# orybkin/video-gcp

Hardware: AMD Instinct MI355X
Metric: predicted frames/sec, 64x64x3 seq_len=80 gcp_tree (posterior forward + all loss terms, model(inputs) and model.loss() of train.py:157-159, batch-stat BatchNorm) (higher is better)
Workload: dtype f32 (encoder / decoder convs and the tree GEMMs from 512 rows: split-f16 MFMA with f32 accumulate, f32-equivalent; everything else exact f32 MFMA)

## Files before the change

include/gcpx.h:

```cpp
#ifndef GCPX_H
#define GCPX_H

#include <stdint.h>

#ifdef __cplusplus
extern "C" {
#endif

#define GCPX_VERSION 1

typedef enum gcpx_status {
    GCPX_OK = 0,
    GCPX_ERR_INVALID_ARG = -1,
    GCPX_ERR_UNSUPPORTED = -2,
    GCPX_ERR_HIP = -3,
    GCPX_ERR_COMM = -4
} gcpx_status;

typedef enum gcpx_act { GCPX_ACT_NONE = 0, GCPX_ACT_LRELU = 1, GCPX_ACT_TANH = 2 } gcpx_act;

int gcpx_version(void);
const char* gcpx_last_error(void);
int gcpx_conv_grid(void);

typedef struct gcpx_conv_src {
    const float* ptr;
    const float* scale;
    const float* shift;
    int32_t C;
    int32_t frame_div;
    int32_t act;
    int32_t _pad;
} gcpx_conv_src;

typedef enum gcpx_head_mode {
    GCPX_HEAD_RAW = 0,
    GCPX_HEAD_DLM_MEAN = 1,
    GCPX_HEAD_DLM_BOTH = 2,
    GCPX_HEAD_TANH_NCHW = 3,
    GCPX_HEAD_DLM_NLL = 4,
    GCPX_HEAD_DLM_NLL_GRAD = 5
} gcpx_head_mode;

typedef struct gcpx_conv_args {
    gcpx_conv_src src[2];
    int32_t nsrc;
    int32_t F;
    int32_t Hin, Win;
    int32_t Hout, Wout;
    int32_t Cin;
    int32_t Cout;
    int32_t out_pitch;
    int32_t upsample;
    int32_t out_act;
    int32_t head_mode;
    const float* wpk;
    const float* bias;
    float* out;
    float* images;
    float* stats_partial;
    const int32_t* raw_row_map;
    const int32_t* src_row_map;
    const int32_t* src_row_frames;
    int32_t n_src_rows;
    int32_t w_split_log2;
    const void* wpk_split;
    const int32_t* w_split_log2_dev;
    int32_t split_layout;
    int32_t nll_rows;
    const float* nll_target;
    float* nll_partial;
    const float* nll_row_weight;
    float nll_scale;
    int32_t _pad3;
    float* images_rows;
    int64_t images_rows_dup;
    const float* bwd_r;
    const float *bwd_scale, *bwd_shift, *bwd_mean, *bwd_rstd;
    const float* addend;
    int32_t addend_frame_div;
    int32_t _pad4;
} gcpx_conv_args;

typedef enum gcpx_split_layout { GCPX_SPLIT_PLAIN = 0, GCPX_SPLIT_ROWFOLD = 1, GCPX_SPLIT_HEAD32 = 2 } gcpx_split_layout;

int gcpx_conv3x3(const gcpx_conv_args* a, void* stream);
int gcpx_conv3x3_grid(const gcpx_conv_args* a);
int gcpx_conv4x4s2(const gcpx_conv_args* a, void* stream);
int gcpx_conv4x4s2_grid(void);
int gcpx_conv4x4s2_image(const float* x, const float* wpk, const float* bias, float* out,
                         int32_t F, int32_t Hin, int32_t Win, int32_t Cout, int32_t out_act, void* stream);

int gcpx_bn_finalize(const float* partial, int32_t n_partial, int32_t pitch, int32_t C, double count,
                     const float* gamma, const float* beta, float eps, float* scale, float* shift,
                     float* running_mean, float* running_var, float momentum, float* mean_out, float* rstd_out,
                     void* stream);
int gcpx_randn(float* out, int64_t n, uint64_t* state, void* stream);
int gcpx_bn_fold(const float* running_mean, const float* running_var, const float* gamma, const float* beta,
                 float eps, int32_t C, float* scale, float* shift, void* stream);

typedef struct gcpx_row_src {
    const float* ptr;
    const int32_t* rowidx;
    const float* scale;
    const float* shiftv;
    int64_t sb, sr;
    int32_t width;
    int32_t shift;
    int32_t act;
    int32_t cmod;
} gcpx_row_src;

typedef enum gcpx_gemm_epi {
    GCPX_EPI_NONE = 0,
    GCPX_EPI_LRELU = 1,
    GCPX_EPI_LSTM = 2,
    GCPX_EPI_GAUSS_SAMPLE = 3
} gcpx_gemm_epi;

struct gcpx_lstm_bwd_args;
typedef struct gcpx_gemm_args {
    gcpx_row_src src[6];
    int32_t nsrc;
    int32_t M, N, K, rpb;
    const float* wpk;
    const float* bias;
    float* out;
    int64_t ob, orow;
    int32_t epi;
    int32_t nbatch;
    float* stats_partial;
    const float* c_prev;
    int64_t c_prev_stride;
    float* h_out;
    float* c_out;
    int64_t hb, hrow;
    float* h_copy;
    int64_t z_src_off, z_w_off, z_bias_off, z_out_off;
    float* gates_out;
    const void* wpk_split;
    const int32_t* w_split_log2_dev;
    int32_t w_split_log2;
    int32_t _pad_split;
    void* x_planes;
    int32_t* x_exp;
    int64_t x_planes_bytes;
    const struct gcpx_lstm_bwd_args* lstm_bwd;
} gcpx_gemm_args;

int gcpx_gemm(const gcpx_gemm_args* a, void* stream);
int gcpx_gemm_planes_workspace(int32_t M, int32_t K, int32_t nbatch, int64_t* planes_bytes, int64_t* n_exp);
int gcpx_gemm_group_dims(const gcpx_gemm_args* host_table, int32_t n, int32_t* dims, int32_t* total_blocks);
int gcpx_gemm_group(const gcpx_gemm_args* dev_table, const int32_t* dev_dims, int32_t n, int32_t total_blocks, void* stream);
int gcpx_gemm_row_blocks(int32_t M, int32_t N);

typedef enum gcpx_mlp_epi { GCPX_MLP_PLAIN = 0, GCPX_MLP_GAUSS = 1,
                             GCPX_MLP_TANH = 2  } gcpx_mlp_epi;

typedef struct gcpx_mlp_args {
    gcpx_row_src src[6];
    int32_t nsrc;
    int32_t M, rpb;
    int32_t in_dim, mid, n_mid, out_dim;
    const float* w_in;
    const float* b_in;
    const float* w_mid;
    const float* b_mid;
    const float* gn_gamma;
    const float* gn_beta;
    const float* w_out;
    const float* b_out;
    float gn_eps;
    float lrelu_slope;
    int32_t epi;
// ... 420 lines not shown
```

video-gcp_amd/forward_plan.py:

```python
import ctypes as C
import os
from contextlib import contextmanager

import torch

from . import packing as pk
from . import runtime as rt
from .hparams import GCPHParams
from .params import init_params, encoder_layers, encoder_skip_layers, decoder_layers
from .plan_ops import _Plan, _addr, N_LANES


class ForwardPlanMixin:

    def _plan_encoder(self, plan, tag, x_ptr, F, out_ptr, out_ob, out_orow, out_rpb):
        hp, P, lib = self._hp, self.pk, self.lib
        G = lib.gcpx_conv4x4s2_grid()
        S = hp.img_sz
        skip_idx = encoder_skip_layers(hp)
        skips = {}
        a0 = self._buf(f"{tag}.a0", (F, S // 2, S // 2, hp.ngf))
        enc_rec = dict(F=F, x_ptr=x_ptr, a0=a0, r={}, out=(out_ptr, out_ob, out_orow, out_rpb))
        plan.rec[f"enc:{tag}"] = enc_rec
        plan.add(f"enc.input:{tag}", lib.gcpx_conv4x4s2_image, x_ptr, P["enc.input.w"].data_ptr(),
                 P["enc.input.b"].data_ptr(), a0.data_ptr(), F, S, S, hp.ngf, rt.ACT_LRELU)
        prev = (a0.data_ptr(), hp.ngf, 1, None, None, rt.ACT_NONE)
        if 0 in skip_idx:
            skips[0] = (a0, hp.ngf, None, None, rt.ACT_NONE)
        res = S // 2
        for li, (name, cin, cout, norm) in enumerate(self._enc_layers[1:], start=1):
            r = self._buf(f"{tag}.r{li}", (F, res // 2, res // 2, cout))
            enc_rec["r"][li] = r
            stats = self._buf(f"{tag}.st{li}", (G, 2, cout)) if self.training else None
            a = self._conv_args([prev], F, res, res, res // 2, res // 2, cout, cout, P[f"enc.{name}.w"],
                                P[f"enc.{name}.b"], r, stats=stats)
            self._set_split(a, f"enc.{name}")
            plan.keep.append(a)
            plan.add(f"enc.{name}:{tag}", lib.gcpx_conv4x4s2, C.byref(a))
            res //= 2
            scale, shift = self._bn(plan, f"{tag}.bn{li}", f"encoder.net.{name}.norm", cout, stats, G, cout,
                                    F * res * res)
            prev = (r.data_ptr(), cout, 1, scale, shift, rt.ACT_LRELU)
            if li in skip_idx:
                skips[li] = (r, cout, scale, shift, rt.ACT_LRELU)
        assert res == 4
        ctop = self._c_top
        src = self._rowsrc(prev[0], 16 * ctop, 16 * ctop, 16 * ctop, scale=prev[3], shiftv=prev[4], act=prev[5], cmod=ctop)
        src.sb, src.sr = out_rpb * 16 * ctop, 16 * ctop
        self._gemm(plan, f"enc.head:{tag}", [src], F, hp.nz_enc, out_rpb, P["enc.head.w"], P["enc.head.b"],
                   out=out_ptr, ob=out_ob, orow=out_orow)
        return skips

    def _plan_seq_encoder(self, plan, tag, prefix, enc_traj, out, B):
        hp, P, lib = self._hp, self.pk, self.lib
        T, nz = hp.max_seq_len, hp.nz_enc
        y1 = self._buf(f"{tag}.y1", (B * T, hp.nz_mid))
        y2 = self._buf(f"{tag}.y2", (B * T, hp.nz_mid))
        taps = lambda t, w, **kw: [self._rowsrc(t.data_ptr(), T * w, w, w, shift=d, **kw) for d in (-1, 0, 1)]
        self._gemm(plan, f"{tag}.input", taps(enc_traj, nz), B * T, hp.nz_mid, T, P[f"{tag}.input.w"], P[f"{tag}.input.b"],
                   out=y1.data_ptr(), ob=T * hp.nz_mid, orow=hp.nz_mid, epi=rt.EPI_LRELU)
        assert hp.conv_inf_enc_layers == 1
        nrb = lib.gcpx_gemm_row_blocks(B * T, hp.nz_mid)
        st = self._buf(f"{tag}.st", (nrb, 2, hp.nz_mid)) if self.training else None
        self._gemm(plan, f"{tag}.pyramid-0", taps(y1, hp.nz_mid), B * T, hp.nz_mid, T, P[f"{tag}.pyramid-0.w"],
                   P[f"{tag}.pyramid-0.b"], out=y2.data_ptr(), ob=T * hp.nz_mid, orow=hp.nz_mid, stats=st)
        sc, sh = self._bn(plan, f"{tag}.bn", f"{prefix}.net.pyramid-0.norm", hp.nz_mid, st, nrb, hp.nz_mid, B * T)
        self._gemm(plan, f"{tag}.head", taps(y2, hp.nz_mid, scale=sc, shiftv=sh, act=rt.ACT_LRELU, cmod=hp.nz_mid),
                   B * T, nz, T, P[f"{tag}.head.w"], P[f"{tag}.head.b"], out=out.data_ptr(), ob=T * nz, orow=nz)

    def _plan_attention(self, plan, l, W, el, er, M, n, B, Kp, Vp, tin):
        hp, lib = self._hp, self.lib
        T, nz, dk = hp.max_seq_len, hp.nz_enc, hp.nz_attn_key
        li = l if hp.untied_layers else 0
        qin = self._buf(f"attn.qin{l}", (M, dk))
        self._mlp(plan, f"attn.query{l}", W["attn.query"], [el, er], M, n, out=qin.data_ptr(), ob=n * dk, orow=dk)
        dense = lambda t, w: self._rowsrc(t.data_ptr(), 0, w, w)
        qp = self._buf(f"attn.q{l}", (M, dk))
        self._gemm(plan, f"attn.q_proj{l}", [dense(qin, dk)], M, dk, M, W["attn.q_proj.w"], W["attn.q_proj.b"],
                   out=qp.data_ptr(), ob=0, orow=dk)
        o = self._buf(f"attn.o{l}", (M, nz))
        gamma = self._buf(f"attn.gamma{l}", (M, T))
        temp = self.sd[f"tree_module.tree_modules.{li}.inference.attention.attention_layers.0.temperature"]
        plan.add(f"attn{l}", lib.gcpx_attention, qp.data_ptr(), _addr(Kp, li * B * T * dk), _addr(Vp, li * B * T * nz), None,
                 tin["end_ind"].data_ptr(), temp.data_ptr(), o.data_ptr(), gamma.data_ptr(), M, n, T, dk, nz, hp.n_attention_heads)
        raw = self._buf(f"attn.raw{l}", (M, nz))
        self._gemm(plan, f"attn.out_proj{l}", [dense(o, nz)], M, nz, M, W["attn.out_proj.w"], W["attn.out_proj.b"],
                   out=raw.data_ptr(), ob=0, orow=nz)
        et = self._buf(f"attn.e_tilde{l}", (M, nz))
        self._gemm(plan, f"attn.out{l}", [dense(raw, nz)], M, nz, M, W["attn.out.w"], W["attn.out.b"], out=et.data_ptr(), ob=0, orow=nz)
        plan.rec.setdefault("gamma", {})[l] = gamma
        plan.rec.setdefault("e_tilde", {})[l] = et
        plan.rec.setdefault("attn", {})[l] = dict(qin=qin, qp=qp, o=o, raw=raw, gamma=gamma, et=et, M=M, n=n, li=li, temp=temp)
        return self._rowsrc(et.data_ptr(), n * nz, nz, nz)

    def _plan_decoder_features(self, plan, e_src, F, rpb, skips):
        hp, P, lib = self._hp, self.pk, self.lib
        ctop = self._c_top
        d0 = self._buf("dec.d0", (F, 4, 4, ctop))
        plan.rec["dec"] = dict(F=F, rpb=rpb, e_src=e_src, d0=d0, blocks=[], skips=skips)
        nrb = lib.gcpx_gemm_row_blocks(F, 16 * ctop)
        st = self._buf("dec.st0", (nrb, 2, 16 * ctop)) if self.training else None
        self._gemm(plan, "dec.input", [e_src], F, 16 * ctop, rpb, P["dec.input.w"], P["dec.input.b"], out=d0.data_ptr(),
                   ob=rpb * 16 * ctop, orow=16 * ctop, stats=st)
        sc, sh = self._bn(plan, "dec.bn0", "decoder.net.input.norm", ctop, st, nrb, 16 * ctop, F * 16)
        prev = (d0.data_ptr(), ctop, 1, sc, sh, rt.ACT_LRELU)
        res = 4
        for name, c_prev, c_skip, skip_idx, cout in decoder_layers(hp):
            srcs = [prev]
            if skip_idx >= 0:
                t, C_, ssc, ssh, sact = skips[skip_idx]
                assert C_ == c_skip and t.shape[1] == res
                srcs.append((t.data_ptr(), C_, rpb, ssc, ssh, sact))
            o = self._buf(f"dec.{name}", (F, 2 * res, 2 * res, cout))
            cpad = (cout + 15) // 16 * 16
            hoist = (skip_idx >= 0 and rpb > 1 and F % rpb == 0 and self.split_f16 and cout in (32, 64) and c_prev % 32 == 0 and
                     c_skip % 32 == 0 and f"dec.{name}" in self.pk_split and "fold" not in self.pk_split[f"dec.{name}"] and
                     os.environ.get("GCPX_NO_SKIP_HOIST") is None)
            addend = None
            if hoist:
                addend = self._buf(f"dec.{name}.skip", (F // rpb, 2 * res, 2 * res, cout))
                t, C_, ssc, ssh, sact = skips[skip_idx]
# ... 35 lines not shown
        nz, nv, H, SD = hp.nz_enc, hp.nz_vae, hp.nz_mid_lstm, hp.lstm_state_dim
        PS = 2 ** L + 1
        plan = _Plan(lib)
        G = lib.gcpx_conv_grid()
        def plan_aux_indices():
            AUXK = ("inv_t0", "inv_t1", "cost_start_idx", "cost_end_idx")
            plan.add("aux_sample_indices", lib.gcpx_aux_sample_indices_gauss, tin["end_ind"].data_ptr(), tin["aux_n"].data_ptr(), B,
                     hp.inv_mdl_temp_dist, *[tin[k].data_ptr() for k in AUXK])
        if "aux_n" in tin and pred_len:
            plan_aux_indices()

        E = self._buf("E", (B, PS, nz))
        Hid = self._buf("Hid", (B, PS, SD))
        Z = self._buf("Z", (B, PS, nv))
        PZ = self._buf("PZ", (B, PS, 2 * nv))
        QZ = self._buf("QZ", (B, PS, 2 * nv))
        node_t = self._buf("node_t", (B, N), torch.int32)
        leave = self._buf("leave", (B, N), torch.int32)
        f2n = self._buf("frame2node", (B, T), torch.int32)
        etrow = self._buf("etilde_row", (B * N,), torch.int32)
        seq_len = self._buf("seq_len", (B,), torch.int32)
        kept_idx = self._buf("kept_idx", (B, T), torch.int32)
        node2row = self._buf("node2row", (B, N), torch.int32)

        adaptive, attentive = hp.adaptive, hp.attentive_inference
        if adaptive:
            kept_idx = self._buf("kept_idx", (B, N), torch.int32)
        def plan_bookkeeping():
            if not adaptive:
                plan.add("balanced_binding", lib.gcpx_balanced_binding, tin["end_ind"].data_ptr(), B, L, T, node_t.data_ptr(),
                         leave.data_ptr(), f2n.data_ptr(), etrow.data_ptr(), seq_len.data_ptr(), node2row.data_ptr())
                plan.add("compact_index", lib.gcpx_compact_index, leave.data_ptr(), B, N, T, kept_idx.data_ptr())
                r2f = self._buf("row2frame", (B * T,), torch.int32)
                if self._head_grad_fused(key) or self._rows_direct(key):
                    plan.add("row2frame", lib.gcpx_index_inverse, node2row.data_ptr(), B * N, r2f.data_ptr(), B * T)
                if self._head_grad_fused(key):
                    S_ = hp.img_sz
                    dMD = self._buf("bw.dMD", (B * T, S_, S_, self._head_pitch))
                    plan.add("zero_unmapped", lib.gcpx_zero_unmapped_rows, dMD.data_ptr(), S_ * S_ * self._head_pitch, r2f.data_ptr(), B * T)

        enc_traj = inf_enc = None
        plan.fork([1, 2])
        traj_first = os.environ.get("GCPX_ENC_ORDER") != "small_first"
        def plan_traj_encoder():
            nonlocal enc_traj, inf_enc
            plan.lane = 0
            if has_traj:
                enc_traj = self._buf("enc_traj", (B * T, nz))
                self._plan_encoder(plan, "traj", tin["traj_seq"].data_ptr(), B * T, enc_traj.data_ptr(), T * nz, nz, T)
                if hp.seq_enc == "none":
                    inf_enc = enc_traj
                else:
                    inf_enc = self._buf("inf_enc_seq", (B * T, nz))
                    self._plan_seq_encoder(plan, "seq", "inf_encoder", enc_traj, inf_enc, B)
                if attentive:
                    dk = hp.nz_attn_key
                    n_mod = L if hp.untied_layers else 1
                    if hp.seq_enc == "none":
                        kenc = enc_traj
                    else:
                        kenc = self._buf("inf_key_enc", (B * T, nz))
                        self._plan_seq_encoder(plan, "kseq", "inf_key_encoder.0", enc_traj, kenc, B)
                    keys = self._buf("inf_enc_key_seq", (B * T, dk))
                    dense = lambda t, w: self._rowsrc(t.data_ptr(), 0, w, w)
                    self._gemm(plan, "kseq.key", [dense(kenc, nz)], B * T, dk, B * T, P["kseq.key.w"], P["kseq.key.b"],
                               out=keys.data_ptr(), ob=0, orow=dk)
                    Kp = self._buf("attn.K", (n_mod, B * T, dk))
                    Vp = self._buf("attn.V", (n_mod, B * T, nz))
                    self._gemm(plan, "attn.k_proj", [dense(keys, dk)], B * T, dk, B * T, P["attn.k_proj.w"], P["attn.k_proj.b"],
                               out=Kp.data_ptr(), ob=0, orow=dk, batch=(n_mod, 0, P["attn.k_proj.w"][0].numel(), dk, B * T * dk))
                    self._gemm(plan, "attn.v_proj", [dense(inf_enc, nz)], B * T, nz, B * T, P["attn.v_proj.w"], P["attn.v_proj.b"],
                               out=Vp.data_ptr(), ob=0, orow=nz, batch=(n_mod, 0, P["attn.v_proj.w"][0].numel(), nz, B * T * nz))
                    plan.rec["attn_kv"] = dict(Kp=Kp, Vp=Vp, keys=keys, kenc=kenc, n_mod=n_mod)

        if traj_first:
            plan_traj_encoder()
        plan.lane = 1
        if "rng_all" in tin:
            plan.add("randn", lib.gcpx_randn, tin["rng_all"].data_ptr(), tin["rng_all"].numel(), self._buf("rng_state", (2,), torch.int64).data_ptr())
            if "aux_n" in tin and not pred_len:
                plan.wait(2, 1)
        skips = self._plan_encoder(plan, "I0", tin["I_0"].data_ptr(), B, _addr(E), PS * nz, 0, 1)
        plan.lane = 2
        if not pred_len:
            if "aux_n" in tin:
                plan_aux_indices()
            plan_bookkeeping()
        if hp.attach_cost_mdl and hp.run_cost_mdl and train_aux and self._has_aux_training:
            gt = self._buf("cost_target", (B,))
            rows = hp.input_nc * hp.img_sz
            plan.add("path_cost", lib.gcpx_path_cost, tin["traj_seq"].data_ptr(), tin["cost_start_idx"].data_ptr(),
                     tin["cost_end_idx"].data_ptr(), B, T, rows, hp.img_sz, self._buf("cost_partial", (B, rows)).data_ptr(), gt.data_ptr())
        self._plan_encoder(plan, "Ig", tin["I_g"].data_ptr(), B, _addr(E, 2 ** L * nz), PS * nz, 0, 1)
        outs = {}
        e0 = lambda: self._rowsrc(_addr(E), PS * nz, 0, nz)
        eg = lambda: self._rowsrc(_addr(E, 2 ** L * nz), PS * nz, 0, nz)
        if hp.regress_length and not pred_len:
            plan.wait(2, 1)
            logits = self._buf("seq_len_logits", (B, T))
            self._mlp(plan, "length_pred", P["length_pred"], [e0(), eg()], B, 1, out=logits.data_ptr(), ob=T, orow=0)
            outs["seq_len_logits"] = logits
        if not traj_first:
            plan_traj_encoder()
        plan.lane = 0
        plan.join([1, 2])

        if hp.regress_length and pred_len:
            logits = self._buf("seq_len_logits", (B, T))
            self._mlp(plan, "length_pred", P["length_pred"], [e0(), eg()], B, 1, out=logits.data_ptr(), ob=T, orow=0)
            outs["seq_len_logits"] = logits
            plan.add("sample_length", lib.gcpx_sample_length, logits.data_ptr(), tin["len_u"].data_ptr(), B, T, 2, tin["end_ind"].data_ptr())
            plan_bookkeeping()

        side_merge = False
        for l in range(L):
            W = P[f"tree{l if hp.untied_layers else 0}"]
            s = 2 ** (L - 1 - l)
            n = 2 ** l
            M = B * n
            nodeoff = lambda w: s * w
            el = lambda: self._rowsrc(_addr(E), PS * nz, 2 * s * nz, nz)
            er = lambda: self._rowsrc(_addr(E, 2 * s * nz), PS * nz, 2 * s * nz, nz)
            pz_out = (_addr(PZ, nodeoff(2 * nv)), PS * 2 * nv, 2 * s * 2 * nv)
            z_map = (_addr(Z, nodeoff(nv)), PS * nv, 2 * s * nv)
            nl = hp.n_lstm_layers
            merged = self._buf(f"merged{l}", (M, 2 * nl * H))

            def plan_merge(lv=l, group=None):
                s_, n_ = 2 ** (L - 1 - lv), 2 ** lv
                Wl = P[f"tree{lv if hp.untied_layers else 0}"]
                mg = self._buf(f"merged{lv}", (B * n_, 2 * nl * H))
                if hp.tree_lstm == "sum":
                    for side, mode in ((0, 0), (2 * s_ * SD, 1)):
                        plan.add(f"merge{lv}.{mode}", lib.gcpx_rows_strided, _addr(mg), n_ * SD, SD, _addr(Hid, side), PS * SD, 2 * s_ * SD,
                                 B, n_, SD, mode)
                    return
                if hp.tree_lstm == "linear":
                    h1 = self._rowsrc(_addr(Hid), PS * SD, 2 * s_ * SD, SD)
                    h2 = self._rowsrc(_addr(Hid, 2 * s_ * SD), PS * SD, 2 * s_ * SD, SD)
                    self._gemm(plan, f"merge{lv}", [h1, h2], B * n_, SD, n_, Wl["proj.w"], Wl["proj.b"], out=_addr(mg), ob=n_ * SD, orow=SD,
                               group=group)
                    return
                h1 = self._rowsrc(_addr(Hid), PS * SD, 2 * s_ * SD, H)
                h2 = self._rowsrc(_addr(Hid, 2 * s_ * SD), PS * SD, 2 * s_ * SD, H)
                self._gemm(plan, f"merge{lv}", [h1, h2], B * n_, H, n_, Wl["proj.w"], Wl["proj.b"], out=_addr(mg),
                           ob=n_ * 2 * nl * H, orow=2 * nl * H, batch=(2 * nl, H, Wl["proj.w"][0].numel(), H, H), group=group)

            merge_with_predictors = not has_z and not sample_prior and hp.tree_lstm not in ("sum", "")
            if has_z:
                g = (_addr(tin["z"], (s - 1) * nv), N * nv, 2 * s * nv) + z_map
                self._mlp(plan, f"prior{l}", W["prior"], [el(), er()], M, n, out=pz_out[0], ob=pz_out[1], orow=pz_out[2], gauss=g)
            elif sample_prior:
                g = (_addr(tin["eps"], (n - 1) * nv), N * nv, nv) + z_map
                self._mlp(plan, f"prior{l}", W["prior"], [el(), er()], M, n, out=pz_out[0], ob=pz_out[1], orow=pz_out[2], gauss=g)
            else:
                pq = []
                self._mlp(plan, f"prior{l}", W["prior"], [el(), er()], M, n, out=pz_out[0], ob=pz_out[1], orow=pz_out[2], group=pq)
                if attentive:
                    et = self._plan_attention(plan, l, W, el(), er(), M, n, B, plan.rec["attn_kv"]["Kp"], plan.rec["attn_kv"]["Vp"], tin)
                else:
                    et = self._rowsrc(inf_enc.data_ptr(), 0, nz, nz, rowidx=etrow[B * (n - 1):])
                g = (_addr(tin["eps"], (n - 1) * nv), N * nv, nv) + z_map
                self._mlp(plan, f"posterior{l}", W["q"], [el(), er(), et], M, n, out=_addr(QZ, nodeoff(2 * nv)),
                          ob=PS * 2 * nv, orow=2 * s * 2 * nv, gauss=g, group=pq)
                mg = []
                if l > 0 and merge_with_predictors and not side_merge:
                    plan_merge(l, group=mg)
                self._mlp_group(plan, f"prior+posterior{l}", pq, gemm=(mg[0] if mg else None))
                if side_merge:
                    plan.join([1])
                    side_merge = False
            zs = lambda: self._rowsrc(z_map[0], z_map[1], z_map[2], nv)
            if not hp.tree_lstm:
                srcs = [el(), er(), zs()] + ([e0(), eg()] if hp.context_every_step else [])
                self._mlp(plan, f"subgoal{l}", W["sg"], srcs, M, n, out=_addr(E, nodeoff(nz)), ob=PS * nz, orow=2 * s * nz, tanh=True)
                continue
# ... 290 lines not shown
```

video-gcp_amd/runtime.py:

```python
import ctypes as C
import os

_HERE = os.path.dirname(os.path.abspath(__file__))
LIB_PATH = os.path.join(_HERE, "libgcpx.so")

ACT_NONE, ACT_LRELU, ACT_TANH = 0, 1, 2
HEAD_RAW, HEAD_DLM_MEAN, HEAD_DLM_BOTH, HEAD_TANH_NCHW, HEAD_DLM_NLL, HEAD_DLM_NLL_GRAD = 0, 1, 2, 3, 4, 5
SPLIT_PLAIN, SPLIT_ROWFOLD, SPLIT_HEAD32 = 0, 1, 2
EPI_NONE, EPI_LRELU, EPI_LSTM, EPI_GAUSS_SAMPLE = 0, 1, 2, 3
MLP_PLAIN, MLP_GAUSS, MLP_TANH = 0, 1, 2

vp = C.c_void_p
i32 = C.c_int32
i64 = C.c_int64


class ConvSrc(C.Structure):
    _fields_ = [("ptr", vp), ("scale", vp), ("shift", vp), ("C", i32), ("frame_div", i32), ("act", i32), ("_pad", i32)]


class ConvArgs(C.Structure):
    _fields_ = [("src", ConvSrc * 2), ("nsrc", i32), ("F", i32), ("Hin", i32), ("Win", i32), ("Hout", i32),
                ("Wout", i32), ("Cin", i32), ("Cout", i32), ("out_pitch", i32), ("upsample", i32), ("out_act", i32),
                ("head_mode", i32), ("wpk", vp), ("bias", vp), ("out", vp), ("images", vp), ("stats_partial", vp),
# ... 24 lines not shown
                ("hb", i64), ("hrow", i64), ("h_copy", vp), ("z_src_off", i64), ("z_w_off", i64),
                ("z_bias_off", i64), ("z_out_off", i64), ("gates_out", vp),
                ("wpk_split", vp), ("w_split_log2_dev", vp), ("w_split_log2", i32), ("_pad_split", i32),
                ("x_planes", vp), ("x_exp", vp), ("x_planes_bytes", i64), ("lstm_bwd", vp)]


class MlpArgs(C.Structure):
    _fields_ = [("src", RowSrc * 6), ("nsrc", i32), ("M", i32), ("rpb", i32), ("in_dim", i32), ("mid", i32),
                ("n_mid", i32), ("out_dim", i32), ("w_in", vp), ("b_in", vp), ("w_mid", vp), ("b_mid", vp),
                ("gn_gamma", vp), ("gn_beta", vp), ("w_out", vp), ("b_out", vp), ("gn_eps", C.c_float),
                ("lrelu_slope", C.c_float), ("epi", i32), ("out_split", i32), ("out", vp), ("ob", i64), ("orow", i64),
                ("oblk", i64), ("eps", vp), ("eb", i64), ("erow", i64), ("z", vp), ("zb", i64), ("zrow", i64), ("save", vp)]


class MlpBwdDx(C.Structure):
    _fields_ = [("wT", vp), ("out", vp), ("ob", i64), ("orow", i64), ("width", i32), ("_pad", i32)]


class MlpBwdArgs(C.Structure):
    _fields_ = [("dout", vp), ("save", vp), ("wT_out", vp), ("wT_mid", vp * 4), ("gn_gamma", vp * 4), ("gn_beta", vp * 4),
                ("du", vp * 5), ("gn_partial", vp * 4), ("dx", MlpBwdDx * 4), ("ldo", i64), ("M", i32), ("rpb", i32),
                ("mid", i32), ("n_mid", i32), ("out_pad", i32), ("ndx", i32), ("gn_eps", C.c_float), ("lrelu_slope", C.c_float)]


class SplitPackDesc(C.Structure):
    _fields_ = [("src", vp), ("idx", vp), ("out", vp), ("log2_out", vp), ("n", i32), ("_pad", i32)]


class WgradArgs(C.Structure):
    _fields_ = [("dy", vp), ("x", vp), ("rowidx", vp), ("frame_map", vp), ("scale", vp), ("shiftv", vp), ("out", vp),
                ("ldy", i64), ("sb", i64), ("sr", i64), ("ldw", i64), ("dy_sb", i64), ("R", i32), ("N", i32), ("n_valid", i32),
                ("K", i32), ("mode", i32), ("Cin", i32), ("H", i32), ("W", i32), ("rpb", i32), ("shift", i32),
                ("act", i32), ("cmod", i32), ("k_off", i32), ("accumulate", i32), ("partial", i32), ("nsplit", i32),
                ("dy_rpb", i32), ("nbatch", i32), ("dbias", vp), ("dbias2", vp), ("z_dy_off", i64), ("z_x_off", i64),
                ("z_out_off", i64), ("z_bias_off", i64), ("split_f16", i32), ("_pad_split", i32)]


class LstmBwdArgs(C.Structure):
    _fields_ = [("gates", vp), ("c_prev", vp), ("c_new", vp), ("dh_dense", vp), ("dh_pos", vp), ("dc_pos", vp),
                ("dgates", vp), ("dc_prev", vp), ("c_prev_stride", i64), ("pb", i64), ("prow", i64), ("dh_stride", i64),
                ("dcp_stride", i64), ("M", i32), ("H", i32), ("rpb", i32), ("_pad", i32)]


class TreeAccumSrc(C.Structure):
    _fields_ = [("ptr", vp), ("ld", i64), ("off_left", i32), ("off_right", i32), ("off_ctx0", i32), ("off_ctxg", i32),
                ("dst_col", i32), ("_pad", i32)]


class TreeAccumArgs(C.Structure):
    _fields_ = [("src", TreeAccumSrc * 6), ("dst", vp), ("dst_sb", i64), ("slot_stride", i64), ("nsrc", i32), ("B", i32),
                ("n", i32), ("width", i32)]


class ActBwdArgs(C.Structure):
    _fields_ = [("da", vp), ("add", vp), ("r", vp), ("scale", vp), ("shift", vp), ("mean", vp), ("rstd", vp), ("dy", vp),
                ("stats_partial", vp), ("ldc", i64), ("c_off", i32), ("up", i32), ("fsum", i32), ("act", i32), ("F", i32),
                ("H", i32), ("W", i32), ("C", i32)]


class PanelTile(C.Structure):
    _fields_ = [("kind", i32), ("src", i32), ("index", i32), ("length", i32), ("flags", i32), ("nb", i32), ("nf", i32),
                ("h", i32), ("w", i32), ("tile_w", i32), ("n0", i32), ("n_b", i32), ("n_f", i32), ("r0", i32), ("r_b", i32),
                ("r_f", i32), ("c0", i32), ("c_b", i32), ("c_f", i32), ("index_off", i32), ("index_stride", i32),
                ("index_count", i32), ("fill", C.c_float), ("_pad", i32), ("off", i64), ("s_b", i64), ("s_f", i64), ("s_c", i64),
                ("s_y", i64)]


PANEL_MAX_SRCS = 16
PANEL_IMAGE, PANEL_GREY, PANEL_GREY_ADD, PANEL_FILL = 0, 1, 2, 3
PANEL_RESCALE, PANEL_LENGTH_STRICT, PANEL_INDEX_FRAME, PANEL_INDEX_I64, PANEL_LENGTH_I64 = 1, 2, 4, 8, 16

WG_ROWS, WG_CONV1D, WG_CONV3X3, WG_CONV4X4S2 = 0, 1, 2, 3
WMAP_LINEAR, WMAP_CONV, WMAP_CONVT = 0, 1, 2

SYMBOLS = [
    ("gcpx_version", C.c_int, []),
    ("gcpx_last_error", C.c_char_p, []),
    ("gcpx_conv_grid", C.c_int, []),
    ("gcpx_conv3x3", C.c_int, [C.POINTER(ConvArgs), vp]),
    ("gcpx_conv3x3_grid", C.c_int, [C.POINTER(ConvArgs)]),
    ("gcpx_conv4x4s2", C.c_int, [C.POINTER(ConvArgs), vp]),
    ("gcpx_conv4x4s2_grid", C.c_int, []),
    ("gcpx_conv4x4s2_image", C.c_int, [vp, vp, vp, vp, i32, i32, i32, i32, i32, vp]),
    ("gcpx_bn_finalize", C.c_int, [vp, i32, i32, i32, C.c_double, vp, vp, C.c_float, vp, vp, vp, vp, C.c_float, vp, vp, vp]),
    ("gcpx_bn_fold", C.c_int, [vp, vp, vp, vp, C.c_float, i32, vp, vp, vp]),
    ("gcpx_randn", C.c_int, [vp, i64, vp, vp]),
    ("gcpx_gemm", C.c_int, [C.POINTER(GemmArgs), vp]),
    ("gcpx_gemm_row_blocks", C.c_int, [i32, i32]),
    ("gcpx_gemm_planes_workspace", C.c_int, [i32, i32, i32, vp, vp]),
    ("gcpx_mlp", C.c_int, [C.POINTER(MlpArgs), vp]),
    ("gcpx_balanced_binding", C.c_int, [vp, i32, i32, i32, vp, vp, vp, vp, vp, vp, vp]),
    ("gcpx_dlm_nll", C.c_int, [vp, vp, vp, vp, i32, i32, i32, i32, vp]),
    ("gcpx_gauss_nll", C.c_int, [vp, vp, vp, vp, i32, i32, vp]),
    ("gcpx_kl_gauss", C.c_int, [vp, vp, i32, i32, i32, i64, i64, C.c_float, vp, i64, vp, vp]),
    ("gcpx_gauss_sample", C.c_int, [vp, i64, i64, vp, i64, i64, vp, i64, i64, i32, i32, i32, vp]),
    ("gcpx_seq_index", C.c_int, [vp, i32, i32, vp, vp, vp]),
    ("gcpx_fill_zero", C.c_int, [vp, i64, vp]),
    ("gcpx_copy_rows", C.c_int, [vp, vp, i32, i32, i64, i64, i64, vp]),
    ("gcpx_loss_combine", C.c_int, [C.POINTER(LossArgs), vp]),
    ("gcpx_loss_pre", C.c_int, [C.POINTER(LossArgs), vp, vp, i32, i32, i64, i64, C.c_float, vp, i64, vp, vp]),
    ("gcpx_loss_final", C.c_int, [C.POINTER(LossArgs), vp]),
    ("gcpx_gather_rows", C.c_int, [vp, vp, vp, i32, i32, i32, i32, i64, vp]),
    ("gcpx_gather_rows_rest", C.c_int, [vp, vp, vp, i32, i32, i32, i32, i64, vp, vp]),
    ("gcpx_compact_index", C.c_int, [vp, i32, i32, i32, vp, vp]),
    ("gcpx_seq_pairs", C.c_int, [vp, vp, vp, vp, i32, i32, i32, vp]),
    ("gcpx_rollout_cost", C.c_int, [vp, i64, vp, vp, i64, vp, i32, i32, i32, i32, i32, C.c_float, vp]),
    ("gcpx_masked_row_sum", C.c_int, [vp, vp, vp, i32, i32, vp]),
    ("gcpx_wgrad", C.c_int, [C.POINTER(WgradArgs), vp]),
    ("gcpx_wgrad_classify", C.c_int, [C.POINTER(WgradArgs), i32, C.POINTER(C.c_int32), C.POINTER(C.c_int32)]),
    ("gcpx_wgrad_group", C.c_int, [vp, vp, i32, i32, i32, vp]),
    ("gcpx_wgrad_conv3x3", C.c_int, [vp, i32, vp, i32, i32, i32, i32, i32, vp, i32, vp]),
    ("gcpx_wgrad_conv3x3_split", C.c_int, [vp, i32, vp, i32, i32, i32, i32, i32, vp, i32, vp]),
    ("gcpx_wgrad_conv3x3_split_up", C.c_int, [vp, i32, C.POINTER(ConvArgs), i32, vp, i32, vp]),
    ("gcpx_wgrad_conv3x3_split_src", C.c_int, [vp, i32, vp, vp, vp, vp, i32, i32, i32, i32, i32, vp, vp, i32, vp]),
    ("gcpx_wgrad_image4x4s2", C.c_int, [vp, vp, vp, vp, i32, i32, vp, i32, vp]),
    ("gcpx_split_pack_group", C.c_int, [vp, i32, vp]),
    ("gcpx_split_pack_group2", C.c_int, [vp, i32, vp, vp]),
    ("gcpx_wgrad_reduce", C.c_int, [vp, i32, i32, i32, vp, i32, i32, i32, i32, vp, i64, i32, i32, vp]),
    ("gcpx_colsum", C.c_int, [vp, i64, i32, i32, i32, i64, i32, vp, vp, vp, i32, vp]),
    ("gcpx_reduce_partials", C.c_int, [vp, i32, i64, i32, vp, i32, vp]),
    ("gcpx_lstm_bwd", C.c_int, [C.POINTER(LstmBwdArgs), vp]),
    ("gcpx_mlp_bwd", C.c_int, [C.POINTER(MlpBwdArgs), vp]),
    ("gcpx_mlp_bwd_group", C.c_int, [C.POINTER(MlpBwdArgs), i32, vp]),
    ("gcpx_mlp_bwd_blocks", C.c_int, [i32]),
    ("gcpx_gn_lrelu_bwd", C.c_int, [vp, vp, vp, vp, vp, vp, i32, i32, i32, C.c_float, C.c_float, vp]),
    ("gcpx_gn_bwd_blocks", C.c_int, [i32]),
    ("gcpx_tanh_bwd_rows", C.c_int, [vp, vp, vp, i64, i64, i32, i32, i32, vp]),
    ("gcpx_lrelu_bwd", C.c_int, [vp, vp, vp, i64, C.c_float, vp]),
    ("gcpx_kl_bwd", C.c_int, [vp, vp, vp, vp, i32, i32, i32, i64, i64, C.c_float, C.c_float, vp]),
    ("gcpx_kl_bwd_weighted", C.c_int, [vp, vp, vp, vp, i32, i32, i32, i64, i64, C.c_float, C.c_float, vp, i64, vp]),
    ("gcpx_kl_bwd_scheduled", C.c_int, [vp, vp, vp, vp, i32, i32, i32, i64, i64, C.c_float, C.c_float, vp, i64, vp, vp]),
    ("gcpx_rows_strided", C.c_int, [vp, i64, i64, vp, i64, i64, i32, i32, i32, i32, vp]),
    ("gcpx_latent_bwd", C.c_int, [vp, vp, vp, i64, i64, vp, i64, i64, vp, i64, vp, i64, vp, vp, i32, i32, i32, vp]),
    ("gcpx_tree_accum", C.c_int, [C.POINTER(TreeAccumArgs), vp]),
    ("gcpx_timestep_scatter", C.c_int, [vp, i64, i64, vp, vp, i32, i32, i32, i32, vp]),
    ("gcpx_add_rows", C.c_int, [vp, i64, i64, vp, vp, i32, i32, i32, vp]),
    ("gcpx_zero_unmapped_rows", C.c_int, [vp, i64, vp, i32, vp]),
    ("gcpx_index_offset", C.c_int, [vp, vp, i32, i32, i32, vp]),
    ("gcpx_index_inverse", C.c_int, [vp, i32, vp, i32, vp]),
    ("gcpx_act_bwd", C.c_int, [C.POINTER(ActBwdArgs), vp]),
    ("gcpx_act_bwd_blocks", C.c_int, []),
    ("gcpx_act_skip_bwd", C.c_int, [C.POINTER(ActBwdArgs), vp, i32, i32, i32, vp]),
    ("gcpx_bn_bwd_finalize", C.c_int, [vp, i32, i32, C.c_double, vp, vp, vp, vp, vp, i32, vp]),
    ("gcpx_bn_bwd_apply", C.c_int, [vp, vp, vp, vp, vp, i64, i32, vp]),
    ("gcpx_conv_stage", C.c_int, [C.POINTER(ConvArgs), vp]),
    ("gcpx_col2im4x4s2", C.c_int, [vp, vp, i32, i32, i32, i32, vp]),
    ("gcpx_im2col_image", C.c_int, [vp, vp, i32, i32, i32, vp]),
    ("gcpx_dlm_nll_bwd", C.c_int, [vp, vp, vp, C.c_float, vp, vp, vp, i32, i32, i32, i32, vp]),
    ("gcpx_loss_heads_bwd", C.c_int, [C.POINTER(LossArgs), vp, vp, vp, vp]),
    ("gcpx_image_metrics", C.c_int, [vp, vp, vp, vp, vp, i32, i32, i32, i32, i32, vp, vp, vp]),
    ("gcpx_topn_accumulate", C.c_int, [vp, i32, i32, i32, i32, i32, vp, vp, vp, i32, vp, vp, vp, i32, vp, vp, i32, vp, i32, vp, i64,
                                        vp]),
    ("gcpx_gemm_group_dims", C.c_int, [vp, i32, vp, vp]),
    ("gcpx_gemm_group", C.c_int, [vp, vp, i32, i32, vp]),
    ("gcpx_mlp_group_dims", C.c_int, [vp, i32, vp, vp]),
    ("gcpx_mlp_group", C.c_int, [vp, vp, i32, i32, i32, vp]),
    ("gcpx_mlp_group_gemm_supported", C.c_int, [C.POINTER(GemmArgs), i32, i32]),
    ("gcpx_mlp_group_gemm", C.c_int, [vp, vp, i32, i32, i32, C.POINTER(GemmArgs), vp]),
    ("gcpx_loss_aux_heads_bwd", C.c_int, [C.POINTER(LossArgs), vp, vp, vp]),
    ("gcpx_aux_sample_indices", C.c_int, [vp, vp, i32, i32, vp, vp, vp, vp, vp]),
    ("gcpx_aux_sample_indices_gauss", C.c_int, [vp, vp, i32, i32, vp, vp, vp, vp, vp]),
    ("gcpx_aux_index_rows", C.c_int, [vp, vp, vp, vp, i32, i32, i32, vp, vp]),
    ("gcpx_path_cost", C.c_int, [vp, vp, vp, i32, i32, i32, i32, vp, vp, vp]),
    ("gcpx_sample_length", C.c_int, [vp, vp, i32, i32, i32, vp, vp]),
    ("gcpx_repack", C.c_int, [vp, vp, vp, vp, i64, vp]),
    ("gcpx_split_pack", C.c_int, [vp, vp, i32, vp, vp, vp]),
# ... 91 lines not shown
```

Before: 477,100.

## Fuse encoder input conv with first 4x4s2 conv in one LDS-resident kernel

Adds a kernel that computes the first image conv (3->16) into LDS and immediately runs the second 4x4 stride-2 conv (16->32, split-f16 MFMA) from LDS, with per-frame exponent scaling, BN stat partials and double-buffered image prefetch. The intermediate a0 activation no longer needs a global write and read-back unless it is a skip or saved for backward. It also adds an env-gated option to reorder the Ig encoder before the small lane-2 bookkeeping ops. The cost is a large LDS footprint per block and half the usual grid, which limits occupancy.

```diff
diff --git a/include/gcpx.h b/include/gcpx.h
--- a/include/gcpx.h
+++ b/include/gcpx.h
@@ -90,6 +90,9 @@
 int gcpx_conv4x4s2_grid(void);
 int gcpx_conv4x4s2_image(const float* x, const float* wpk, const float* bias, float* out,
                          int32_t F, int32_t Hin, int32_t Win, int32_t Cout, int32_t out_act, void* stream);
+int gcpx_conv4x4s2_pair_supported(const gcpx_conv_args* layer2, int32_t Hin, int32_t Win);
+int gcpx_conv4x4s2_pair(const float* x, const float* wpk1, const float* bias1, int32_t out_act1, float* a0,
+                        const gcpx_conv_args* layer2, int32_t max_blocks, void* stream);
 
 int gcpx_bn_finalize(const float* partial, int32_t n_partial, int32_t pitch, int32_t C, double count,
                      const float* gamma, const float* beta, float eps, float* scale, float* shift,
diff --git a/video-gcp_amd/csrc/conv_enc_pair.hip b/video-gcp_amd/csrc/conv_enc_pair.hip
--- /dev/null
+++ b/video-gcp_amd/csrc/conv_enc_pair.hip
@@ -0,0 +1,261 @@
+#include "common.h"
+
+#include <cstdlib>
+
+namespace {
+
+typedef _Float16 h8 __attribute__((ext_vector_type(8)));
+
+__device__ __forceinline__ f32x4 mfma32h(h8 a, h8 b, f32x4 c) {
+    return __builtin_amdgcn_mfma_f32_16x16x32_f16(a, b, c, 0, 0, 0);
+}
+
+struct PairCfg {
+    static constexpr int HIN = 64, PITCH = HIN + 8, ROWS = HIN + 2, PLANE = ROWS * PITCH, IMG_BYTES = 3 * PLANE * 4;
+    static constexpr int MH = HIN / 2, NG1 = MH * MH / 16, F4 = 3 * HIN * HIN / 4, PRE = F4 / 256;
+    static constexpr int CIN = 16, COUT = 32, HOUT = MH / 2, CT = 2, WP = 2, WC = 2, PIXB = CIN * 4 + 16, PGW = 8, NSTEP = 8;
+    static constexpr int FRAME_PIX = MH * MH, FRAME_BYTES = FRAME_PIX * PIXB;
+    static constexpr int RED_OFF = IMG_BYTES + FRAME_BYTES;
+    static constexpr int LDS_BYTES = RED_OFF + (WP * 2 * CT * 16 + 4) * 4;
+    static_assert(IMG_BYTES % 16 == 0 && F4 % 256 == 0 && LDS_BYTES <= 160 * 1024, "LDS layout");
+};
+
+__global__ void __launch_bounds__(256) conv4x4s2_pair_kernel(const float* __restrict__ x, const float* __restrict__ wpk1,
+                                                             const float* __restrict__ bias1, const int out_act1, float* __restrict__ a0,
+                                                             const gcpx_conv_args a, const int nrows, const float one, const float zero) {
+    using Cfg = PairCfg;
+    constexpr int HIN = Cfg::HIN, PITCH = Cfg::PITCH, PLANE = Cfg::PLANE, MH = Cfg::MH, NG1 = Cfg::NG1, F4 = Cfg::F4, PRE = Cfg::PRE;
+    constexpr int COUT = Cfg::COUT, HOUT = Cfg::HOUT, CT = Cfg::CT, WP = Cfg::WP, PIXB = Cfg::PIXB, PGW = Cfg::PGW, NSTEP = Cfg::NSTEP;
+    constexpr int FRAME_PIX = Cfg::FRAME_PIX, C8 = Cfg::CIN / 8;
+    extern __shared__ float4 pair_smem4[];
+    float* img = reinterpret_cast<float*>(pair_smem4);
+    char* lds = reinterpret_cast<char*>(pair_smem4) + Cfg::IMG_BYTES;
+    float* red = reinterpret_cast<float*>(reinterpret_cast<char*>(pair_smem4) + Cfg::RED_OFF);
+    float* wmax = red + WP * 2 * CT * 16;
+    const int tid = threadIdx.x, lane = tid & 63, wave = tid >> 6;
+    const int wp = wave % WP, wc = wave / WP;
+    const int j = lane & 15, q = lane >> 4;
+    const int F = a.F;
+
+    for (int i = tid; i < 3 * 2 * PITCH; i += 256) {
+        const int pl = i / (2 * PITCH), r = (i / PITCH) % 2, c = i % PITCH;
+        img[pl * PLANE + (r ? HIN + 1 : 0) * PITCH + c] = 0.f;
+    }
+    for (int i = tid; i < 3 * Cfg::ROWS * 2; i += 256) {
+        const int pl = i / (Cfg::ROWS * 2), r = (i / 2) % Cfg::ROWS, c = (i & 1) ? HIN + 4 : 3;
+        img[pl * PLANE + r * PITCH + c] = 0.f;
+    }
+    float w1[12];
+#pragma unroll
+    for (int t = 0; t < 12; ++t) w1[t] = wpk1[t * 64 + lane];
+    const float4 bv1 = *reinterpret_cast<const float4*>(bias1 + q * 4);
+    h8 w2[NSTEP][2];
+    {
+        const char* wbase = reinterpret_cast<const char*>(a.wpk_split) + (size_t)wc * 2048 + lane * 16;
+#pragma unroll
+        for (int s = 0; s < NSTEP; ++s) {
+            w2[s][0] = *reinterpret_cast<const h8*>(wbase + (size_t)s * CT * 2048);
+            w2[s][1] = *reinterpret_cast<const h8*>(wbase + (size_t)s * CT * 2048 + 1024);
+        }
+    }
+    const float4 bv2 = *reinterpret_cast<const float4*>(a.bias + wc * 16 + q * 4);
+    const int ew = a.w_split_log2_dev ? __builtin_amdgcn_readfirstlane(*a.w_split_log2_dev) : a.w_split_log2;
+
+    int base[PGW], pin_[PGW];
+    unsigned vmask[PGW];
+#pragma unroll
+    for (int pt = 0; pt < PGW; ++pt) {
+        const int pin = (wp + pt * WP) * 16 + j;
+        const int oy = pin / HOUT, ox = pin % HOUT;
+        pin_[pt] = pin;
+        base[pt] = ((2 * oy - 1) * MH + 2 * ox - 1) * PIXB;
+        unsigned m = 0;
+        for (int k = 0; k < 4; ++k) {
+            if (2 * oy - 1 + k >= 0 && 2 * oy - 1 + k < MH) m |= 1u << k;
+            if (2 * ox - 1 + k >= 0 && 2 * ox - 1 + k < MH) m |= 16u << k;
+        }
+        vmask[pt] = m;
+    }
+
+    const f32x4* xsrc = reinterpret_cast<const f32x4*>(x) + tid;
+    int ioff[PRE];
+#pragma unroll
+    for (int k = 0; k < PRE; ++k) {
+        const int i = k * 256 + tid;
+        const int pl = i / (HIN * HIN / 4), rem = i % (HIN * HIN / 4);
+        const int y = rem / (HIN / 4), x4 = rem % (HIN / 4);
+        ioff[k] = pl * PLANE + (y + 1) * PITCH + 4 + 4 * x4;
+    }
+    f32x4 pre[PRE];
+#define PAIR_IMG_LOAD(frame)                                                         \
+    _Pragma("unroll") for (int k = 0; k < PRE; ++k) pre[k] = xsrc[(size_t)(frame) * F4 + k * 256]
+#define PAIR_IMG_STORE()                                                             \
+    _Pragma("unroll") for (int k = 0; k < PRE; ++k) *reinterpret_cast<f32x4*>(img + ioff[k]) = pre[k]
+
+    int f = blockIdx.x;
+    PAIR_IMG_LOAD(f);
+    PAIR_IMG_STORE();
+    __syncthreads();
+    for (; f < F; f += gridDim.x) {
+        float amax = 0.f;
+        for (int g = wave; g < NG1; g += 4) {
+            const int p = g * 16 + j;
+            const int oy = p / MH, ox = p % MH;
+            const float* bp = img + (2 * oy) * PITCH + 3 + 2 * ox + q;
+            f32x4 acc = f32x4{0, 0, 0, 0};
+#pragma unroll
+            for (int ci = 0; ci < 3; ++ci)
+#pragma unroll
+                for (int ky = 0; ky < 4; ++ky) acc = mfma16(w1[ci * 4 + ky], bp[ci * PLANE + ky * PITCH], acc);
+            f32x4 v = acc;
+            v[0] += bv1.x; v[1] += bv1.y; v[2] += bv1.z; v[3] += bv1.w;
+            if (out_act1 == GCPX_ACT_LRELU) {
+                v[0] = lrelu(v[0], 0.2f); v[1] = lrelu(v[1], 0.2f); v[2] = lrelu(v[2], 0.2f); v[3] = lrelu(v[3], 0.2f);
+            }
+            if (a0) *reinterpret_cast<float4*>(a0 + ((size_t)f * FRAME_PIX + p) * 16 + q * 4) = make_float4(v[0], v[1], v[2], v[3]);
+            float4 s;
+            s.x = fmaf(v[0], one, zero); s.y = fmaf(v[1], one, zero); s.z = fmaf(v[2], one, zero); s.w = fmaf(v[3], one, zero);
+            amax = fmaxf(amax, fmaxf(fmaxf(fabsf(s.x), fabsf(s.y)), fmaxf(fabsf(s.z), fabsf(s.w))));
+            *reinterpret_cast<float4*>(lds + p * PIXB + 16 * q) = s;
+        }
+#pragma unroll
+        for (int m = 1; m < 64; m <<= 1) amax = fmaxf(amax, __shfl_xor(amax, m));
+        if (lane == 0) wmax[wave] = amax;
+        __syncthreads();
+        const bool has_next = f + (int)gridDim.x < F;
+        PAIR_IMG_LOAD(has_next ? f + (int)gridDim.x : f);
+
+        amax = fmaxf(fmaxf(wmax[0], wmax[1]), fmaxf(wmax[2], wmax[3]));
+        int ex = 14 + 127 - (int)((__float_as_uint(amax) >> 23) & 0xff);
+        ex = __builtin_amdgcn_readfirstlane(amax > 0.f ? max(-100, min(min(100, 126 - ew), ex)) : min(100, 126 - ew));
+        const float sx2 = __uint_as_float((unsigned)(127 + ex) << 23);
+        for (int i = tid; i < FRAME_PIX * C8; i += 256) {
+            const int c8 = i % C8, pix = i / C8;
+            char* p = lds + pix * PIXB + 32 * c8;
+            const float4 v0 = *reinterpret_cast<const float4*>(p), v1 = *reinterpret_cast<const float4*>(p + 16);
+            const float fv[8] = {v0.x * sx2, v0.y * sx2, v0.z * sx2, v0.w * sx2, v1.x * sx2, v1.y * sx2, v1.z * sx2, v1.w * sx2};
+            h8 p1, p2;
+#pragma unroll
+            for (int e = 0; e < 8; ++e) {
+                p1[e] = (_Float16)fv[e];
+                p2[e] = (_Float16)fmaf((float)p1[e], -1.f, fv[e]);
+            }
+            *reinterpret_cast<h8*>(p) = p1;
+            *reinterpret_cast<h8*>(p + 16) = p2;
+        }
+        __syncthreads();
+
+        f32x4 acc[PGW];
+#pragma unroll
+        for (int pt = 0; pt < PGW; ++pt) acc[pt] = f32x4{0, 0, 0, 0};
+#pragma unroll
+        for (int step = 0; step < NSTEP; ++step) {
+            const int tap = 2 * step + (q >> 1), grp = q & 1;
+            const int ky = tap >> 2, kx = tap & 3;
+            const int tapoff = (ky * MH + kx) * PIXB + grp * 32;
+            h8 b[PGW][2];
+#pragma unroll
+            for (int pt = 0; pt < PGW; ++pt) {
+                const bool ok = ((vmask[pt] >> ky) & 1u) && ((vmask[pt] >> (4 + kx)) & 1u);
+                const char* p = lds + (ok ? base[pt] + tapoff : 0);
+                const h8 t0 = *reinterpret_cast<const h8*>(p), t1 = *reinterpret_cast<const h8*>(p + 16);
+                const h8 z = {0, 0, 0, 0, 0, 0, 0, 0};
+                b[pt][0] = ok ? t0 : z;
+                b[pt][1] = ok ? t1 : z;
+            }
+#pragma unroll
+            for (int pt = 0; pt < PGW; ++pt) acc[pt] = mfma32h(w2[step][1], b[pt][0], acc[pt]);
+#pragma unroll
+            for (int pt = 0; pt < PGW; ++pt) acc[pt] = mfma32h(w2[step][0], b[pt][1], acc[pt]);
+#pragma unroll
+            for (int pt = 0; pt < PGW; ++pt) acc[pt] = mfma32h(w2[step][0], b[pt][0], acc[pt]);
+        }
+        const float inv = __uint_as_float((unsigned)(127 - ex - ew) << 23);
+        f32x4 st1 = f32x4{0, 0, 0, 0}, st2 = f32x4{0, 0, 0, 0};
+#pragma unroll
+        for (int pt = 0; pt < PGW; ++pt) {
+            float* op = a.out + ((size_t)f * HOUT * HOUT + pin_[pt]) * COUT;
+            const int c = wc * 16 + q * 4;
+            f32x4 v = acc[pt];
+            v[0] = fmaf(v[0], inv, bv2.x); v[1] = fmaf(v[1], inv, bv2.y); v[2] = fmaf(v[2], inv, bv2.z); v[3] = fmaf(v[3], inv, bv2.w);
+            if (a.out_act == GCPX_ACT_LRELU) {
+                v[0] = lrelu(v[0], 0.2f); v[1] = lrelu(v[1], 0.2f); v[2] = lrelu(v[2], 0.2f); v[3] = lrelu(v[3], 0.2f);
+            }
+            *reinterpret_cast<float4*>(op + c) = make_float4(v[0], v[1], v[2], v[3]);
+            if (a.stats_partial) { st1 += v; st2 += v * v; }
+        }
+        if (a.stats_partial) {
+#pragma unroll
+            for (int r = 0; r < 4; ++r) {
+                const float s1 = row16_sum(st1[r]);
+                const float s2 = row16_sum(st2[r]);
+                if (j == 0) {
+                    const int c = wc * 16 + q * 4 + r;
+                    red[(wp * 2 + 0) * CT * 16 + c] = s1;
+                    red[(wp * 2 + 1) * CT * 16 + c] = s2;
+                }
+            }
+        }
+        if (has_next) { PAIR_IMG_STORE(); }
+        __syncthreads();
+        if (a.stats_partial && tid < 2 * CT * 16) {
+            const int which = tid / (CT * 16), c = tid % (CT * 16);
+            float sum = 0.f;
+#pragma unroll
+            for (int w_ = 0; w_ < WP; ++w_) sum += red[(w_ * 2 + which) * CT * 16 + c];
+            a.stats_partial[((size_t)f * 2 + which) * CT * 16 + c] = sum;
+        }
+    }
+    if (a.stats_partial && tid < 2 * CT * 16)
+        for (int r = F + blockIdx.x; r < nrows; r += gridDim.x) a.stats_partial[(size_t)r * 2 * CT * 16 + tid] = 0.f;
+}
+#undef PAIR_IMG_LOAD
+#undef PAIR_IMG_STORE
+
+bool pair_supported(const gcpx_conv_args* a, int Hin, int Win) {
+    if (!a || Hin != 64 || Win != 64) return false;
+    if (a->nsrc != 1 || a->src[0].frame_div != 1 || a->src[0].C != 16) return false;
+    if (a->Cin != 16 || a->Cout != 32 || a->out_pitch != 32 || a->Hin != 32 || a->Win != 32 || a->Hout != 16 || a->Wout != 16) return false;
+    if (!a->wpk_split || a->split_layout != GCPX_SPLIT_PLAIN || getenv("GCPX_ENC_NOSPLIT")) return false;
+    if (a->src[0].scale || a->src[0].shift || a->src[0].act != GCPX_ACT_NONE) return false;
+    if (a->src_row_map) return false;
+    return a->F > 0 && a->F <= gcpx_conv4x4s2_grid();
+}
+
+}
+
+extern "C" int gcpx_conv4x4s2_pair_supported(const gcpx_conv_args* layer2, int32_t Hin, int32_t Win) {
+    return pair_supported(layer2, Hin, Win) ? 1 : 0;
+}
+
+extern "C" int gcpx_conv4x4s2_pair(const float* x, const float* wpk1, const float* bias1, int32_t out_act1, float* a0,
+                                   const gcpx_conv_args* layer2, int32_t max_blocks, void* stream_) {
+    hipStream_t stream = reinterpret_cast<hipStream_t>(stream_);
+    const gcpx_conv_args* a = layer2;
+    GCPX_CHECK_ARG(a != nullptr, "null args");
+    GCPX_CHECK_ARG(x && wpk1 && bias1 && a->wpk && a->bias && a->out && a->F > 0, "null pointer / F <= 0");
+    GCPX_CHECK_ARG(out_act1 == GCPX_ACT_NONE || out_act1 == GCPX_ACT_LRELU, "first layer: no activation or LeakyReLU");
+    GCPX_CHECK_ARG(max_blocks >= 0, "max_blocks < 0");
+    if (!pair_supported(a, a->Hin * 2, a->Win * 2)) {
+        gcpx_set_error("conv4x4s2_pair: no fused form (64 x 64 images, 16 -> 32 split-f16 layer in the plain layout reading a0 without "
+                       "scale / activation, F <= %d); F=%d Hin=%d Cin=%d Cout=%d", gcpx_conv4x4s2_grid(), a->F, a->Hin, a->Cin, a->Cout);
+        return GCPX_ERR_UNSUPPORTED;
+    }
+    static bool attr_set = false;
+    if (!attr_set) {
+        hipError_t e = hipFuncSetAttribute(reinterpret_cast<const void*>(conv4x4s2_pair_kernel), hipFuncAttributeMaxDynamicSharedMemorySize,
+                                           PairCfg::LDS_BYTES);
+        if (e != hipSuccess) {
+            gcpx_set_error("conv4x4s2_pair: hipFuncSetAttribute(%d B): %s", PairCfg::LDS_BYTES, hipGetErrorString(e));
+            return GCPX_ERR_HIP;
+        }
+        attr_set = true;
+    }
+    int grid = gcpx_conv_grid() / 2;
+    if (max_blocks > 0 && grid > max_blocks) grid = max_blocks;
+    if (grid > a->F) grid = a->F;
+    hipLaunchKernelGGL(conv4x4s2_pair_kernel, dim3(grid), dim3(256), PairCfg::LDS_BYTES, stream, x, wpk1, bias1, out_act1, a0, *a,
+                       gcpx_conv4x4s2_grid(), 1.f, 0.f);
+    GCPX_CHECK_LAUNCH();
+    return GCPX_OK;
+}
diff --git a/video-gcp_amd/forward_plan.py b/video-gcp_amd/forward_plan.py
--- a/video-gcp_amd/forward_plan.py
+++ b/video-gcp_amd/forward_plan.py
@@ -19,14 +19,10 @@
         S = hp.img_sz
         skip_idx = encoder_skip_layers(hp)
         skips = {}
-        a0 = self._buf(f"{tag}.a0", (F, S // 2, S // 2, hp.ngf))
-        enc_rec = dict(F=F, x_ptr=x_ptr, a0=a0, r={}, out=(out_ptr, out_ob, out_orow, out_rpb))
+        enc_rec = dict(F=F, x_ptr=x_ptr, a0=None, r={}, out=(out_ptr, out_ob, out_orow, out_rpb))
         plan.rec[f"enc:{tag}"] = enc_rec
-        plan.add(f"enc.input:{tag}", lib.gcpx_conv4x4s2_image, x_ptr, P["enc.input.w"].data_ptr(),
-                 P["enc.input.b"].data_ptr(), a0.data_ptr(), F, S, S, hp.ngf, rt.ACT_LRELU)
-        prev = (a0.data_ptr(), hp.ngf, 1, None, None, rt.ACT_NONE)
-        if 0 in skip_idx:
-            skips[0] = (a0, hp.ngf, None, None, rt.ACT_NONE)
+        a0_buf = lambda: self._buf(f"{tag}.a0", (F, S // 2, S // 2, hp.ngf))
+        prev = (None, hp.ngf, 1, None, None, rt.ACT_NONE)
         res = S // 2
         for li, (name, cin, cout, norm) in enumerate(self._enc_layers[1:], start=1):
             r = self._buf(f"{tag}.r{li}", (F, res // 2, res // 2, cout))
@@ -36,7 +32,23 @@
                                 P[f"enc.{name}.b"], r, stats=stats)
             self._set_split(a, f"enc.{name}")
             plan.keep.append(a)
-            plan.add(f"enc.{name}:{tag}", lib.gcpx_conv4x4s2, C.byref(a))
+            if li == 1:
+                pair = os.environ.get("GCPX_ENC_NO_PAIR") is None and lib.gcpx_conv4x4s2_pair_supported(C.byref(a), S, S) == 1
+                a0 = a0_buf() if (not pair or 0 in skip_idx or self.save_for_backward) else None
+                enc_rec["a0"] = a0
+                if a0 is not None:
+                    a.src[0].ptr = a0.data_ptr()
+                    if 0 in skip_idx:
+                        skips[0] = (a0, hp.ngf, None, None, rt.ACT_NONE)
+                if pair:
+                    plan.add(f"enc.input+{name}:{tag}", lib.gcpx_conv4x4s2_pair, x_ptr, P["enc.input.w"].data_ptr(),
+                             P["enc.input.b"].data_ptr(), rt.ACT_LRELU, a0.data_ptr() if a0 is not None else None, C.byref(a), 0)
+                else:
+                    plan.add(f"enc.input:{tag}", lib.gcpx_conv4x4s2_image, x_ptr, P["enc.input.w"].data_ptr(),
+                             P["enc.input.b"].data_ptr(), a0.data_ptr(), F, S, S, hp.ngf, rt.ACT_LRELU)
+                    plan.add(f"enc.{name}:{tag}", lib.gcpx_conv4x4s2, C.byref(a))
+            else:
+                plan.add(f"enc.{name}:{tag}", lib.gcpx_conv4x4s2, C.byref(a))
             res //= 2
             scale, shift = self._bn(plan, f"{tag}.bn{li}", f"encoder.net.{name}.norm", cout, stats, G, cout,
                                     F * res * res)
@@ -238,16 +250,22 @@
                 plan.wait(2, 1)
         skips = self._plan_encoder(plan, "I0", tin["I_0"].data_ptr(), B, _addr(E), PS * nz, 0, 1)
         plan.lane = 2
-        if not pred_len:
-            if "aux_n" in tin:
-                plan_aux_indices()
-            plan_bookkeeping()
-        if hp.attach_cost_mdl and hp.run_cost_mdl and train_aux and self._has_aux_training:
-            gt = self._buf("cost_target", (B,))
-            rows = hp.input_nc * hp.img_sz
-            plan.add("path_cost", lib.gcpx_path_cost, tin["traj_seq"].data_ptr(), tin["cost_start_idx"].data_ptr(),
-                     tin["cost_end_idx"].data_ptr(), B, T, rows, hp.img_sz, self._buf("cost_partial", (B, rows)).data_ptr(), gt.data_ptr())
+        def plan_lane2_small():
+            if not pred_len:
+                if "aux_n" in tin:
+                    plan_aux_indices()
+                plan_bookkeeping()
+            if hp.attach_cost_mdl and hp.run_cost_mdl and train_aux and self._has_aux_training:
+                gt = self._buf("cost_target", (B,))
+                rows = hp.input_nc * hp.img_sz
+                plan.add("path_cost", lib.gcpx_path_cost, tin["traj_seq"].data_ptr(), tin["cost_start_idx"].data_ptr(),
+                         tin["cost_end_idx"].data_ptr(), B, T, rows, hp.img_sz, self._buf("cost_partial", (B, rows)).data_ptr(), gt.data_ptr())
+        ig_first = os.environ.get("GCPX_IG_ORDER") == "first"
+        if not ig_first:
+            plan_lane2_small()
         self._plan_encoder(plan, "Ig", tin["I_g"].data_ptr(), B, _addr(E, 2 ** L * nz), PS * nz, 0, 1)
+        if ig_first:
+            plan_lane2_small()
         outs = {}
         e0 = lambda: self._rowsrc(_addr(E), PS * nz, 0, nz)
         eg = lambda: self._rowsrc(_addr(E, 2 ** L * nz), PS * nz, 0, nz)
diff --git a/video-gcp_amd/runtime.py b/video-gcp_amd/runtime.py
--- a/video-gcp_amd/runtime.py
+++ b/video-gcp_amd/runtime.py
@@ -130,6 +130,8 @@
     ("gcpx_conv4x4s2", C.c_int, [C.POINTER(ConvArgs), vp]),
     ("gcpx_conv4x4s2_grid", C.c_int, []),
     ("gcpx_conv4x4s2_image", C.c_int, [vp, vp, vp, vp, i32, i32, i32, i32, i32, vp]),
+    ("gcpx_conv4x4s2_pair_supported", C.c_int, [C.POINTER(ConvArgs), i32, i32]),
+    ("gcpx_conv4x4s2_pair", C.c_int, [vp, vp, vp, i32, vp, C.POINTER(ConvArgs), i32, vp]),
     ("gcpx_bn_finalize", C.c_int, [vp, i32, i32, i32, C.c_double, vp, vp, C.c_float, vp, vp, vp, vp, C.c_float, vp, vp, vp]),
     ("gcpx_bn_fold", C.c_int, [vp, vp, vp, vp, C.c_float, i32, vp, vp, vp]),
     ("gcpx_randn", C.c_int, [vp, i64, vp, vp]),
```

Measured after the change: 484,500, median of 6. +1.6%, better.
